# biodatageeks/datafusion-bio-functions

Hardware: AMD Instinct MI355X
Metric: overlap-pairs/sec + probe-rows/sec, IntervalJoinExec 100Mx1M (higher is better)
Workload: dtype int32; 1 GPU; join_100Mx1M_24contigs; probe_rows_per_gpu=100000000, build_rows_per_gpu=1000000, contigs=24, pairs_per_gpu=37210484, parallelism=partition-per-gpu x1, gather=False, build_overlap=True

## Files before the change

datafusion-bio-functions_amd/csrc/ivx_capi.hip:

```cpp
#include "ivx_internal.hpp"
#include "ivx_call.hpp"
#include "ivx_where.hpp"
#include <cstdlib>
#include <atomic>
#include <cstring>
#include <mutex>
#include <new>
#include <thread>
#include <condition_variable>
#include <deque>


void ivx_ctx::join_tail()
{
    if (!tail_pending) return;
    (void)hipStreamWaitEvent(stream, tail_ev, 0);
    tail_pending = false;
}

ivx_status ivx_ctx::get_scratch(int slot, size_t bytes, void **out)
{
    if (tail_pending && slot != WS_SORTHIST && slot != WS_T0 && slot != WS_T1 && slot != WS_T2) join_tail();
    ivx_buf &b = scratch[slot];
    if (sub_plan.valid && ((sub_plan.slots >> slot) & 1)) sub_plan.valid = false;
// ... 409 lines not shown
    w[IVX_STATE_JOIN_FILLS_PLANNED] = ctx->join_fills_planned;
    w[IVX_STATE_SUB_FILLS_PLANNED] = ctx->sub_fills_planned;
    for (int i = 0; i < IVX_NSCRATCH; i++) if (ctx->scratch[i].p) w[IVX_STATE_SCRATCH_HELD] |= 1ull << i;
    {
        std::lock_guard<std::mutex> lk(g_pool_mu);
        for (const PoolBuf &b : g_pool) if (b.device == ctx->device) w[IVX_STATE_POOL_FREE]++;
    }
    for (u32 i = 0; i < n_out && i < (u32)IVX_STATE_WORDS; i++) out[i] = w[i];
    return IVX_OK;
}

extern "C" ivx_status ivx_debug_poison(ivx_ctx *ctx, uint32_t word, int what, uint64_t *slots_written)
{
    if (!ctx) return IVX_ERR_INVALID;
    if (slots_written) *slots_written = 0;
    if (word > 1u) return ctx->fail(IVX_ERR_INVALID, "debug_poison: the word is 0 or 1");
    if (ctx->tail_pending) return ctx->fail(IVX_ERR_INVALID, "debug_poison: a build tail is pending");
    IVX_HIP(ctx, hipSetDevice(ctx->device));
    IVX_HIP(ctx, hipStreamSynchronize(ctx->stream));
    hipStream_t st = ctx->stream;
    const auto fill_host = [word](void *p, size_t bytes) { u32 *q = (u32 *)p; for (size_t i = 0; i < bytes / sizeof(u32); i++) q[i] = word; };
    if (what & IVX_POISON_DROP_PLANS) { ctx->sub_plan.valid = false; ctx->join_plan.valid = false; }
    if (what & IVX_POISON_SCRATCH) {
        const u64 keep = (ctx->sub_plan.valid ? ctx->sub_plan.slots : 0) | (ctx->join_plan.valid ? ctx->join_plan.rows.slots : 0);
        u64 wrote = 0;
        for (int i = 0; i < IVX_NSCRATCH; i++) {
            const ivx_buf &b = ctx->scratch[i];
            if (!b.p || ((keep >> i) & 1)) continue;
            IVX_HIP(ctx, hipMemsetD32Async((hipDeviceptr_t)b.p, (int)word, b.cap / sizeof(u32), st));
            wrote |= 1ull << i;
        }
// ... 1420 lines not shown
```

datafusion-bio-functions_amd/csrc/ivx_device.hpp:

```cpp
#pragma once
#include "ivx_internal.hpp"

__device__ __forceinline__ u32 lane_id() { return __builtin_amdgcn_mbcnt_hi(~0u, __builtin_amdgcn_mbcnt_lo(~0u, 0u)); }

__device__ __forceinline__ u32 mask_rank_from(u64 mask, u32 base)
{
    return __builtin_amdgcn_mbcnt_hi((u32)(mask >> 32), __builtin_amdgcn_mbcnt_lo((u32)mask, base));
}

__device__ __forceinline__ u32 mask_rank(u64 mask)
{
    return __builtin_amdgcn_mbcnt_hi((u32)(mask >> 32), __builtin_amdgcn_mbcnt_lo((u32)mask, 0u));
}

template <typename T>
__device__ __forceinline__ void host_store(T *p, T v) { __hip_atomic_store(p, v, __ATOMIC_RELAXED, __HIP_MEMORY_SCOPE_SYSTEM); }

template <int CTRL, int ROWS>
__device__ __forceinline__ u32 dpp0(u32 v) { return (u32)__builtin_amdgcn_update_dpp(0, (int)v, CTRL, ROWS, 0xf, false); }
__device__ __forceinline__ u32 wave_incl_max32(u32 v)
{
    u32 o;
    o = dpp0<0x111, 0xf>(v); v = o > v ? o : v;
    o = dpp0<0x112, 0xf>(v); v = o > v ? o : v;
// ... 19 lines not shown
#pragma unroll
    for (int d = 1; d < IVX_WAVE; d <<= 1) {
        T o = __shfl_up(v, d, IVX_WAVE);
        if (l >= (u32)d) v += o;
    }
    return v;
}

template <typename T>
__device__ __forceinline__ T wave_sum(T v)
{
#pragma unroll
    for (int d = IVX_WAVE / 2; d > 0; d >>= 1) v += __shfl_xor(v, d, IVX_WAVE);
    return v;
}

template <typename T, int NT>
__device__ __forceinline__ T block_excl_scan(T v, T *lds, T *total)
{
    constexpr int NW = NT / IVX_WAVE;
    const u32 l = lane_id();
    const u32 w = threadIdx.x / IVX_WAVE;
    T inc = wave_incl_scan(v);
    if (l == IVX_WAVE - 1) lds[w] = inc;
    __syncthreads();
    if (threadIdx.x == 0) {
        T run = 0;
#pragma unroll
        for (int i = 0; i < NW; i++) { T t = lds[i]; lds[i] = run; run += t; }
        lds[NW] = run;
// ... 30 lines not shown
```

datafusion-bio-functions_amd/csrc/ivx_grid.hip:

```cpp
#include <cstdlib>
#include "ivx_grid.hpp"
#include "ivx_scan.hpp"

namespace {

constexpr int GT = 256;
constexpr u32 KEYS_IN_LDS = 2048;

__global__ void k_init_keystats(i32 *kmin, i32 *kmax, u32 *kcnt, u32 nkeys, ivx_zero_ranges z)
{
    u32 i = blockIdx.x * blockDim.x + threadIdx.x;
    if (i < nkeys) { kmin[i] = INT32_MAX; kmax[i] = INT32_MIN; kcnt[i] = 0; }
    if (blockIdx.x == 0)
        for (int r = 0; r < 3; r++)
            for (u32 j = threadIdx.x; j < z.n[r]; j += blockDim.x) z.p[r][j] = 0;
    for (u32 j = i; j < z.nbig; j += gridDim.x * blockDim.x) z.big[j] = make_uint4(0u, 0u, 0u, 0u);
}

__global__ __launch_bounds__(GT) void k_keystats(const u32 *__restrict__ key, const i32 *__restrict__ v, u64 n,
                                                 u32 nkeys, i32 *kmin, i32 *kmax, u32 *kcnt, u32 *errflag, u32 vs,
                                                 const i32 *__restrict__ vend, u32 *lenhist)
{
    extern __shared__ i32 sh[];
    __shared__ u32 s_len[33];
    if (lenhist && threadIdx.x < 33) s_len[threadIdx.x] = 0;
    const bool priv = nkeys <= KEYS_IN_LDS;
    if (!priv && lenhist) __syncthreads();
    i32 *smin = sh, *smax = sh + nkeys;
    u32 *scnt = (u32 *)(sh + 2 * nkeys);
    if (priv) {
        for (u32 k = threadIdx.x; k < nkeys; k += GT) { smin[k] = INT32_MAX; smax[k] = INT32_MIN; scnt[k] = 0; }
// ... 17 lines not shown
            clcnt++;
        }
        if (k != ck) { flush(); ck = k; ccnt = 0; cmin = INT32_MAX; cmax = INT32_MIN; }
        cmin = x < cmin ? x : cmin; cmax = x > cmax ? x : cmax; ccnt++;
    }
    flush();
    if (lenhist && clcnt) atomicAdd(&s_len[cl], clcnt);
    if (priv) {
        __syncthreads();
        for (u32 k = threadIdx.x; k < nkeys; k += GT)
            if (scnt[k]) { atomicMin(&kmin[k], smin[k]); atomicMax(&kmax[k], smax[k]); atomicAdd(&kcnt[k], scnt[k]); }
    }
    if (lenhist) {
        __syncthreads();
        if (threadIdx.x < 33 && s_len[threadIdx.x]) atomicAdd(&lenhist[threadIdx.x], s_len[threadIdx.x]);
    }
}

__global__ __launch_bounds__(GT) void k_keystats_sorted(const u32 *__restrict__ key, const i32 *__restrict__ v, u64 n, u32 nkeys,
                                                        i32 *kmin, i32 *kmax, u32 *kcnt, u32 vs)
{
    const u32 k = blockIdx.x * GT + threadIdx.x;
    if (k >= nkeys) return;
    auto lower = [&](u32 x) {
        u64 a = 0, b = n;
        while (a < b) { const u64 m = (a + b) >> 1; if ((key ? key[m] : 0u) < x) a = m + 1; else b = m; }
        return a;
    };
    const u64 lo = lower(k), hi = k + 1 == 0u ? n : lower(k + 1);
    kcnt[k] = (u32)(hi - lo);
// ... 108 lines not shown
}

ivx_status ivx_keystats(ivx_ctx *ctx, const u32 *key, const i32 *v, u64 n, u32 nkeys,
                        i32 *kmin, i32 *kmax, u32 *kcnt, u32 *errflag, u32 vstride)
{
    return ivx_keystats_len(ctx, key, v, n, nkeys, kmin, kmax, kcnt, errflag, vstride, nullptr, nullptr);
}

ivx_status ivx_keystats_len(ivx_ctx *ctx, const u32 *key, const i32 *v, u64 n, u32 nkeys,
                            i32 *kmin, i32 *kmax, u32 *kcnt, u32 *errflag, u32 vstride, const i32 *vend, u32 *lenhist,
                            const ivx_zero_ranges *zero)
{
    hipStream_t st = ctx->stream;
    ivx_zero_ranges z{};
    if (zero) z = *zero;
    u32 igrid = (nkeys + GT - 1) / GT;
    if (z.nbig) { const u32 want = (z.nbig + GT * 8 - 1) / (GT * 8); igrid = igrid > want ? igrid : (want < 256u ? want : 256u); }
    hipLaunchKernelGGL(k_init_keystats, dim3(igrid), dim3(GT), 0, st, kmin, kmax, kcnt, nkeys, z);
    if (n) {
        const u32 grid = ivx_stream_grid(n, GT * 8, 1024);
        const size_t shm = nkeys <= KEYS_IN_LDS ? (size_t)nkeys * 12 : 0;
        hipLaunchKernelGGL(k_keystats, dim3(grid), dim3(GT), shm, st, key, v, n, nkeys, kmin, kmax, kcnt, errflag, vstride, vend, lenhist);
    }
    IVX_HIP(ctx, hipGetLastError());
    return IVX_OK;
}

ivx_status ivx_grid_build(ivx_ctx *ctx, ivx_index *ix, const u32 *key, const i32 *v, u64 n, u32 nkeys, RankGridView *out, bool sorted, u32 vstride)
{
    if (!sorted && vstride != 1) return ctx->fail(IVX_ERR_INVALID, "grid: strided values need a sorted column");
    hipStream_t st = ctx->stream;
    const u64 maxcells = 2 * n + nkeys + 64;
    if (maxcells + 1 >= 0xFFFFFFFFull) return ctx->fail(IVX_ERR_INVALID, "column too large for 32-bit cell ids");
    i32 *origin, *val; u32 *span, *kcnt, *koff, *kbase, *binstart, *hdr;
    IVX_TRY(ivx_index_alloc(ctx, ix, nkeys * sizeof(i32), (void **)&origin));
    IVX_TRY(ivx_index_alloc(ctx, ix, nkeys * sizeof(u32), (void **)&span));
    IVX_TRY(ivx_index_alloc(ctx, ix, nkeys * sizeof(u32), (void **)&kcnt));
    IVX_TRY(ivx_index_alloc(ctx, ix, ((size_t)nkeys + 1) * sizeof(u32), (void **)&koff));
// ... 32 lines not shown
```

datafusion-bio-functions_amd/csrc/ivx_grid.hpp:

```cpp
#pragma once
#include "ivx_device.hpp"

template <int VS = 1>
__device__ __forceinline__ u32 grid_rank_le(const RankGridView &g, u32 sh, u32 k, i32 x)
{
    const u32 cnt = g.kcnt[k];
    const u32 off = g.koff[k];
    if (cnt == 0) return off;
    const i64 d = (i64)x - (i64)g.origin[k];
    if (d < 0) return off;
    if (d > (i64)g.span[k]) return off + cnt;
    const u32 c = g.kbase[k] + (u32)(d >> sh);
    const u32 a = g.binstart[c], b = g.binstart[c + 1];
    u32 r = a;
    for (u32 j = a; j < b; j++) r += g.val[(u64)j * VS] <= x ? 1u : 0u;
    return r;
}

template <int VS = 1>
__device__ __forceinline__ u32 grid_rank_lt(const RankGridView &g, u32 sh, u32 k, i32 x)
{
    if (x == INT32_MIN) return g.koff[k];
    return grid_rank_le<VS>(g, sh, k, x - 1);
}

ivx_status ivx_keystats(ivx_ctx *ctx, const u32 *key, const i32 *v, u64 n, u32 nkeys,
                        i32 *kmin, i32 *kmax, u32 *kcnt, u32 *errflag);
ivx_status ivx_grid_build(ivx_ctx *ctx, ivx_index *ix, const u32 *key, const i32 *v, u64 n, u32 nkeys, RankGridView *out, bool sorted = false,
                          u32 vstride = 1);
ivx_status ivx_keystats(ivx_ctx *ctx, const u32 *key, const i32 *v, u64 n, u32 nkeys,
                        i32 *kmin, i32 *kmax, u32 *kcnt, u32 *errflag, u32 vstride);
struct ivx_zero_ranges { u32 *p[3]; u32 n[3]; uint4 *big = nullptr; u32 nbig = 0; };
ivx_status ivx_keystats_len(ivx_ctx *ctx, const u32 *key, const i32 *v, u64 n, u32 nkeys,
                            i32 *kmin, i32 *kmax, u32 *kcnt, u32 *errflag, u32 vstride, const i32 *vend, u32 *lenhist,
                            const ivx_zero_ranges *zero = nullptr);
```

datafusion-bio-functions_amd/csrc/ivx_internal.hpp:

```cpp
#pragma once
#include <hip/hip_runtime.h>
#include <stdint.h>
#include <atomic>
#include <memory>
#include <string>
#include <vector>
#include "../../include/ivx.h"
#include "../../include/ivx_select.h"
#include "../../include/ivx_nearest.h"

typedef uint8_t u8;
typedef uint32_t u32;
typedef int32_t i32;
typedef uint64_t u64;
typedef int64_t i64;

#define IVX_WAVE 64

struct ivx_buf { void *p = nullptr; size_t cap = 0; };

enum { IVX_NSCRATCH = 56, IVX_NPIN = 4 };

struct ivx_sub_plan {
    bool valid = false;
// ... 124 lines not shown
    WS_GRID0, WS_GRID1, WS_GRID2,
    WS_SORTHIST,
    WS_SA0, WS_SA1, WS_SA2, WS_SB0, WS_SB1, WS_SB2,
    WS_RA0, WS_RA1, WS_RA2, WS_RB0, WS_RB1, WS_RB2,
    WS_T0, WS_T1, WS_T2, WS_T3, WS_T4, WS_T5, WS_T6, WS_T7, WS_T8, WS_T9,
    WS_IN3_KEY, WS_IN3_START, WS_IN3_END, WS_IN3_WEIGHT, WS_IN_KEYLEN,
    WS_IN_TEXTOFF, WS_IN_TEXT
};
static_assert(WS_IN_TEXT < IVX_NSCRATCH, "scratch slot ids must fit the context's slot array");

#ifndef IVX_LSTEP
#define IVX_LSTEP 2
#endif
#define IVX_MAXL (32 / IVX_LSTEP)
#define IVX_SH_MIN 4

struct ivx_ent { i32 s, e; u32 row; };

enum { HDR_SH0 = 0, HDR_NLEV = 1, HDR_NBINS = 2, HDR_CS = 3 , HDR_NREG = 4,
       HDR_RCELLS = 5 , HDR_RMUL_LO = 6, HDR_RMUL_HI = 7 , HDR_LEVCNT = 8 ,
       HDR_FG = 8 + IVX_MAXL , HDR_FBITS = 9 + IVX_MAXL ,
       HDR_PK24 = 10 + IVX_MAXL ,
       HDR_SLOW = 11 + IVX_MAXL ,
       HDR_LBUILD = 12 + IVX_MAXL ,
       HDR_BADKEY = 13 + IVX_MAXL ,
       HDR_WORDS = 14 + IVX_MAXL };
#include "ivx_scalars.hpp"
#define IVX_FBITS_MAX (1u << 24)
#define IVX_MAXREG 255
#define IVX_MAXREG_WIDE 1023
// ... 248 lines not shown
```

datafusion-bio-functions_amd/csrc/ivx_join.hip:

```cpp
#include <cstdlib>
#include <cstring>
#include "ivx_device.hpp"
#include "ivx_grid.hpp"
#include "ivx_join.hpp"

namespace {

constexpr int BT = 256;

constexpr int LB_T = 1024;
constexpr int LB_ROWS = 4;
constexpr u32 LB_TILE = LB_T * LB_ROWS;
constexpr u32 LB_STRIDE = IVX_MAXREG_WIDE + 1;
constexpr u32 LB_CCAP = 8192;
constexpr u32 LB_MAXTILES = 1024;
constexpr int LB_KEEP = (IVX_RP_ECAP + LB_T - 1) / LB_T;
constexpr u64 LB_MIN_ROWS = 1u << 14, LB_MAX_ROWS = (u64)LB_MAXTILES * LB_TILE;
static_assert(LB_STRIDE == LB_T && LB_TILE <= 4096 && LB_CCAP == (1u << IVX_REG_CS_MAX), "k_lbuild_tiles: one table word per thread, 12-bit ranks");
static inline u32 lb_tstride(u32 ntiles) { return ntiles | 1u; }


__device__ __forceinline__ u32 cells_of(u32 cnt, u32 span, u32 sh) { return cnt ? (sh >= 32 ? 1u : (span >> sh) + 1u) : 0u; }

__global__ __launch_bounds__(1024) void k_join_layout(const i32 *kmin, const i32 *kmax, const u32 *kcnt, u32 nkeys, u64 n,
                                                      i32 *origin, u32 *span, u32 *lbase, u32 *hdr, u64 maxcells,
                                                      u32 *kreg, u32 *rkey, const u32 *lenhist, u32 regmax, u32 *fbase, int filter_mode, int lbuild_ok, const u32 *badkey,
                                                      u32 *hmirror)
{
    __shared__ u64 red[1024 / IVX_WAVE + 1];
    __shared__ u32 s_sh0;
    const u32 t = threadIdx.x;
    for (u32 k = t; k < nkeys; k += 1024) {
        u32 c = kcnt[k];
        origin[k] = c ? kmin[k] : 0;
        span[k] = c ? (u32)((i64)kmax[k] - (i64)kmin[k]) : 0u;
    }
    __syncthreads();
    __shared__ u64 s_tot[40];
    __shared__ u64 s_loff[IVX_MAXL + 1];
    const u32 wv = t / IVX_WAVE, ln = lane_id();
    constexpr u32 NWV = 1024 / IVX_WAVE;
    const u64 budget0 = 2 * n + nkeys;
    for (u32 sh = IVX_SH_MIN + wv; sh <= 31; sh += NWV) {
        u64 a = 0;
        for (u32 k = ln; k < nkeys; k += IVX_WAVE) a += cells_of(kcnt[k], span[k], sh);
        a = wave_sum(a);
        if (ln == 0) s_tot[sh] = a;
    }
    __syncthreads();
    __shared__ float s_occ0;
    __shared__ u64 s_cum[34];
    __shared__ float s_cost[32], s_cocc[32];
    __shared__ u32 s_shb;
    if (t <= 32) s_cum[t + 1] = lenhist[t];
    __syncthreads();
    __shared__ u32 s_fg;
    if (t == 0) {
        u32 shb = IVX_SH_MIN;
        while (shb < 31 && s_tot[shb] > budget0) shb++;
        s_shb = shb;
        u32 fg = 0xFFFFFFFFu;
        if (filter_mode != 0 && (u64)nkeys * 34 < IVX_FBITS_MAX / 2) {
            u32 g = IVX_SH_MIN;
            while (g < 31 && s_tot[g] + (u64)nkeys * 34 > IVX_FBITS_MAX) g++;
            const double bits = (double)(s_tot[g] + nkeys);
            double touched = 0.0;
            for (u32 b = 0; b <= 32; b++) touched += (double)s_cum[b + 1] * ((b > g ? (double)(3ull << (b - g)) * 0.25 : 0.0) + 1.5);
            if (n && s_tot[g] + (u64)nkeys * 34 <= IVX_FBITS_MAX && (filter_mode == 2 || touched < 0.15 * bits) && touched < 64.0 * (double)n + 1.0e6) fg = g;
        }
// ... 19 lines not shown
                if (l == 0) { occ0 = occ; cost += 1.f + 2.2f * occ; }
                else if (rows) cost += 8.f + 2.2f * occ * 4.f;
                if (last) break;
                lo_bits = lsh + 1;
            }
        }
        s_cost[t] = cost; s_cocc[t] = occ0;
    }
    __syncthreads();
    if (t == 0) {
        u32 bi = 0;
        for (u32 c = 1; c < 32; c++) if (s_cost[c] < s_cost[bi]) bi = c;
#ifdef IVX_SH_BIAS
        { const int b2 = (int)bi + (IVX_SH_BIAS); bi = b2 < 0 ? 0u : (s_shb + (u32)b2 > 31 ? 31 - s_shb : (u32)b2); }
#endif
        s_sh0 = s_shb + bi; s_occ0 = s_cocc[bi];
    }
    __syncthreads();
    const u32 sh0 = s_sh0;
    u32 nlev = 0;
    for (u32 l = 0; l < IVX_MAXL; l++) { nlev = l + 1; if (sh0 + IVX_LSTEP * l >= 32) break; }
    for (u32 l = wv; l < nlev; l += NWV) {
        const u32 sh = sh0 + IVX_LSTEP * l;
        u64 carry = 0;
        for (u32 k0 = 0; k0 < nkeys; k0 += IVX_WAVE) {
            const u32 k = k0 + ln;
            const u64 c = k < nkeys ? cells_of(kcnt[k], span[k], sh) : 0u;
            const u64 inc = wave_incl_scan(c);
            if (k < nkeys) lbase[(u64)l * nkeys + k] = (u32)(carry + inc - c);
            carry += __shfl(inc, IVX_WAVE - 1, IVX_WAVE);
        }
        if (ln == 0) s_tot[l] = carry;
    }
    __syncthreads();
    if (t == 0) {
        u64 run = 0;
        for (u32 l = 0; l < nlev; l++) { s_loff[l] = run; run += s_tot[l]; }
        hdr[HDR_SH0] = sh0;
        hdr[HDR_NLEV] = nlev;
        hdr[HDR_NBINS] = (u32)(run <= maxcells ? run : maxcells);
    }
    __syncthreads();
    for (u32 l = 1 + wv; l < nlev; l += NWV) {
        const u32 add = (u32)s_loff[l];
        for (u32 k = ln; k < nkeys; k += IVX_WAVE) lbase[(u64)l * nkeys + k] += add;
    }
    for (u32 mid = wv; mid <= 32; mid += NWV) {
        u64 a = 0;
        for (u32 k = ln; k < nkeys; k += IVX_WAVE) {
            const u64 c = cells_of(kcnt[k], span[k], sh0);
            a += mid >= 32 ? (c ? 1u : 0u) : ((c + (1ull << mid) - 1) >> mid);
        }
        a = wave_sum(a);
        if (ln == 0) s_tot[mid] = a;
    }
    __syncthreads();
    u32 clo = 0;
    while (clo < 32 && s_tot[clo] > IVX_MAXREG) clo++;
    if (clo > IVX_REG_CS_MAX && clo <= 32 && s_tot[IVX_REG_CS_MAX] <= IVX_MAXREG2) clo = IVX_REG_CS_MAX;
    u64 R = clo < 32 ? (1ull << clo) : 0;
    bool pow2 = true;
    if (clo < 32 && s_occ0 * (float)R > 0.9f * (float)IVX_RP_ECAP) {
        const float want = 0.85f * (float)IVX_RP_ECAP / s_occ0;
        R = want < 1.f ? 1ull : (u64)want;
        pow2 = false;
    }
    auto regions_for = [&](u64 r) -> u64 {
        u64 a = 0;
        for (u32 k = t; k < nkeys; k += 1024) { const u64 c = cells_of(kcnt[k], span[k], sh0); a += (c + r - 1) / r; }
        return block_sum<u64, 1024>(a, red);
    };
    if (R && nkeys > regmax && regions_for(1ull << 40) > regmax) R = 0;
    if (R) {
        if (!(pow2 && clo < 32 && s_tot[clo] <= regmax)) while (regions_for(R) > regmax) { R *= 2; }
        if (!pow2) {
            u64 mc = 0;
            for (u32 k = t; k < nkeys; k += 1024) { const u64 c = cells_of(kcnt[k], span[k], sh0); mc = c > mc ? c : mc; }
            __shared__ u64 s_mc;
            if (t == 0) s_mc = 0;
            __syncthreads();
            atomicMax((unsigned long long *)&s_mc, (unsigned long long)mc);
            __syncthreads();
            const u64 M = ((1ull << 40) + R - 1) / R;
            if (s_mc * R >= (1ull << 40) || s_mc > (1ull << 63) / M || (R & (R - 1)) == 0) {
                u64 p = 1; while (p * 2 <= R) p *= 2;
                R = p; pow2 = true;
                while (regions_for(R) > regmax) R *= 2;
            }
        }
    }
    u32 cs = 32;
    if (R && pow2) { cs = 0; while ((1ull << cs) < R) cs++; }
    u64 rrun = 0;
    for (u32 k0 = 0; k0 < nkeys; k0 += 1024) {
        const u32 k = k0 + t;
        u64 c = k < nkeys ? cells_of(kcnt[k], span[k], sh0) : 0u;
        c = R ? (c + R - 1) / R : 0;
        u64 tot;
        const u64 ex = block_excl_scan<u64, 1024>(c, red, &tot);
        if (k < nkeys && R) {
            kreg[k] = (u32)(rrun + ex);
            for (u64 r = 0; r < c; r++) rkey[rrun + ex + r] = k;
        }
        rrun += tot;
    }
    {
        const u32 fg = s_fg;
        u64 frun = 0;
        for (u32 k0 = 0; k0 < nkeys; k0 += 1024) {
            const u32 k = k0 + t;
            u64 c = (fg != 0xFFFFFFFFu && k < nkeys && kcnt[k]) ? (u64)(((span[k] >> fg) + 2u + 31u) & ~31u) : 0u;
            u64 tot;
            const u64 ex = block_excl_scan<u64, 1024>(c, red, &tot);
            if (k < nkeys) fbase[k] = (u32)(frun + ex);
            frun += tot;
        }
        if (t == 0) { hdr[HDR_FG] = frun <= IVX_FBITS_MAX ? fg : 0xFFFFFFFFu; hdr[HDR_FBITS] = (u32)frun; }
    }
    if (t == 0) {
        kreg[nkeys] = (u32)rrun;
        hdr[HDR_CS] = pow2 ? cs : 0xFFFFFFFFu;
        hdr[HDR_NREG] = R ? (u32)rrun : 0u;
        hdr[HDR_RCELLS] = (u32)(R > 0xFFFFFFFFull ? 0xFFFFFFFFull : R);
        const u64 M = R ? ((1ull << 40) + R - 1) / R : 0;
        hdr[HDR_RMUL_LO] = (u32)M; hdr[HDR_RMUL_HI] = (u32)(M >> 32);
        hdr[HDR_PK24] = (R && sh0 < 24 && R <= (1ull << (24 - sh0))) ? 1u : 0u;
        hdr[HDR_BADKEY] = *badkey;
        hdr[HDR_LBUILD] = (lbuild_ok && R && R <= LB_CCAP && rrun && rrun <= IVX_MAXREG_WIDE && s_cum[33] == s_cum[sh0 + 1]) ? 1u : 0u;
        static_assert(HDR_WORDS % 2 == 0, "the mirror is written in 8-byte words");
        u32 hv[HDR_WORDS];
#pragma unroll
        for (u32 w = 0; w < HDR_WORDS; w++) hv[w] = hdr[w];
#pragma unroll
        for (u32 w = 0; w < HDR_WORDS; w += 2) host_store((u64 *)hmirror + w / 2, (u64)hv[w] | ((u64)hv[w + 1] << 32));
    }
}

__global__ __launch_bounds__(LB_T) void k_lbuild_tiles(const u32 *__restrict__ key, const i32 *__restrict__ s, const i32 *__restrict__ e, u64 n, u32 nkeys,
                                                     const i32 *origin, const u32 *kreg, u32 *hdr, ivx_ent *__restrict__ rows,
                                                     u32 *__restrict__ tab, u32 tstride, u32 *__restrict__ binstart, u64 nbinwords)
{
    if (hdr[HDR_LBUILD] == 0) {
        for (u64 i = (u64)blockIdx.x * LB_T + threadIdx.x; i < nbinwords; i += (u64)gridDim.x * LB_T) binstart[i] = 0;
        return;
    }
    __shared__ u32 s_cnt[LB_STRIDE];
    __shared__ u32 red[LB_T / IVX_WAVE + 1];
    const u32 t = threadIdx.x;
    s_cnt[t] = 0;
    const u32 sh0 = hdr[HDR_SH0], cs = hdr[HDR_CS];
// ... 384 lines not shown
    IVX_TRY(ivx_index_alloc(ctx, ix, nkeys * sizeof(u32), (void **)&span));
    IVX_TRY(ivx_index_alloc(ctx, ix, nkeys * sizeof(u32), (void **)&kcnt));
    IVX_TRY(ivx_index_alloc(ctx, ix, (size_t)IVX_MAXL * nkeys * sizeof(u32), (void **)&lbase));
    IVX_TRY(ivx_index_alloc(ctx, ix, (maxcells + 1) * sizeof(u32), (void **)&binstart));
    IVX_TRY(ivx_index_alloc(ctx, ix, HDR_WORDS * sizeof(u32), (void **)&hdr));
    IVX_TRY(ivx_index_alloc(ctx, ix, ((size_t)nkeys + 1) * sizeof(u32), (void **)&kreg));
    size_t regcap = (size_t)(n / (IVX_RP_ECAP / 2)) + (size_t)(maxcells >> IVX_REG_CS_MAX) + 2 * (size_t)nkeys + 64;
    regcap = regcap <= IVX_MAXREG + 1 ? (size_t)IVX_MAXREG + 1 : (regcap > (size_t)IVX_MAXREG2 + 1 ? (size_t)IVX_MAXREG2 + 1 : regcap);
    IVX_TRY(ivx_index_alloc(ctx, ix, regcap * sizeof(u32), (void **)&rkey));
    IVX_TRY(ivx_index_alloc(ctx, ix, regcap * sizeof(ivx_regdesc), (void **)&rdesc));
    IVX_TRY(ivx_index_alloc(ctx, ix, (n ? n : 1) * sizeof(ivx_ent), (void **)&ent));
    const size_t fwords = IVX_FBITS_MAX / 32 + 4;
    IVX_TRY(ivx_index_alloc(ctx, ix, nkeys * sizeof(u32), (void **)&fbase));
    IVX_TRY(ivx_index_alloc(ctx, ix, fwords * sizeof(u32), (void **)&fbits));

    i32 *kmin, *kmax; u32 *cellid, *rank, *errflag;
    IVX_TRY(ctx->get_scratch(WS_GRID0, nkeys * sizeof(i32), (void **)&kmin));
    IVX_TRY(ctx->get_scratch(WS_GRID1, nkeys * sizeof(i32), (void **)&kmax));
    const char *benv = getenv("IVX_BUILD");
    const bool lb_try = n >= LB_MIN_ROWS && n <= LB_MAX_ROWS && !(benv && !strcmp(benv, "global"));
    const u32 lb_tiles = lb_try ? (u32)((n + LB_TILE - 1) / LB_TILE) : 0u;
    IVX_TRY(ctx->get_scratch(WS_GRID2, (n ? n : 1) * (lb_try ? sizeof(ivx_ent) : sizeof(u32)), (void **)&cellid));
    const size_t tabbytes = (size_t)lb_tstride(lb_tiles) * LB_STRIDE * sizeof(u32);
    IVX_TRY(ctx->get_scratch(WS_T9, (n ? n : 1) * sizeof(u32) > tabbytes ? (n ? n : 1) * sizeof(u32) : tabbytes, (void **)&rank));
    errflag = ctx->dword<u32>(SC_JOIN_BAD);
    u32 *lenhist = ctx->dword<u32>(SC_JOIN_LENHIST);

    ivx_zero_ranges zr{{errflag, lenhist, hdr}, {1u, (u32)SC_LENHIST_N, (u32)HDR_WORDS}};
    const char *fenv = getenv("IVX_FILTER");
    const int filter_mode = !fenv ? 1 : !strcmp(fenv, "0") ? 0 : !strcmp(fenv, "force") ? 2 : 1;
    static_assert((IVX_FBITS_MAX / 32 + 4) % 4 == 0, "the bitmap is cleared in 16-byte words");
    if (filter_mode) { zr.big = (uint4 *)fbits; zr.nbig = (u32)(fwords / 4); }
    IVX_TRY(ivx_keystats_len(ctx, key, s, n, nkeys, kmin, kmax, kcnt, errflag, 1u, e, lenhist, &zr));
    const u32 grid = ivx_stream_grid(n, BT * 2, 16384);
    u32 *hmirror = ctx->hword<u32>(SC_HDR_MIRROR), *hmirror_d = ctx->hdword<u32>(SC_HDR_MIRROR);
    ctx->hdr_mirror_serial = ix->serial;
    hipLaunchKernelGGL(k_join_layout, dim3(1), dim3(1024), 0, st, kmin, kmax, kcnt, nkeys, n, origin, span, lbase, hdr, maxcells, kreg, rkey, (const u32 *)lenhist, (u32)(regcap - 1), fbase, filter_mode, lb_try ? 1 : 0, (const u32 *)errflag, hmirror_d);
    auto launch_filter = [&]() {
        hipLaunchKernelGGL(k_join_filter, dim3(grid), dim3(BT), 0, st, key, s, e, n, nkeys, (const i32 *)origin, (const u32 *)span, (const u32 *)fbase, (const u32 *)hdr, fbits);
    };
    const bool want_route = ix->kind == IVX_KIND_OVERLAP && n >= (4u << 20);
    overlap = overlap && ctx->overlap && ctx->aux != nullptr && !want_route && n >= (1u << 16);
    if (filter_mode && !overlap) launch_filter();
    hipStream_t tail_st = st;
    struct TailGuard {
        ivx_ctx *c; bool armed = false;
        ~TailGuard() { if (armed) (void)hipStreamSynchronize(c->aux); }
    } guard{ctx};
    bool q_lds = lb_try, q_global = true;
    if (overlap) {
        ctx->join_tail();
        IVX_HIP(ctx, hipEventRecord(ctx->ev_fork, st));
        IVX_HIP(ctx, hipStreamWaitEvent(ctx->aux, ctx->ev_fork, 0));
// ... 77 lines not shown
```

datafusion-bio-functions_amd/csrc/ivx_regions_route.hip:

```cpp
#include "ivx_regions.hpp"

namespace {


constexpr int PA_T = 1024;
#ifndef IVX_PA_I
#define IVX_PA_I 12
#endif
constexpr int PA_I = IVX_PA_I;
constexpr int PA_TILE = PA_T * PA_I;
constexpr u32 NO_REGION = 0xFFFFFFFFu;
constexpr u32 KT_MAX = 256;

struct KeyTab {
    bool lds;
    u32 nkeys, sh0, cs;
    u64 rmul;
};

__device__ __forceinline__ void keytab_load(const JoinIndexView &ix, i32 *s_origin, u32 *s_last, u32 *s_kreg, KeyTab &kt)
{
    kt.nkeys = ix.nkeys; kt.sh0 = ix.hdr[HDR_SH0]; kt.cs = ix.hdr[HDR_CS];
    kt.rmul = (u64)ix.hdr[HDR_RMUL_LO] | ((u64)ix.hdr[HDR_RMUL_HI] << 32);
    kt.lds = ix.nkeys <= KT_MAX;
    if (kt.lds) {
        for (u32 k = threadIdx.x; k < ix.nkeys; k += blockDim.x) {
            s_origin[k] = ix.origin[k];
// ... 1041 lines not shown
```

Before: 38.56 billion overlap-pairs/s.

## Replace atomic build keystats with per-workgroup partials reduced in layout kernel

For small key counts, build-side key statistics (min, max, count, length histogram, bad-key flag) are written as per-workgroup partial arrays instead of being merged with global atomics. The single-block layout kernel then reduces those partials into LDS and reads key tables from LDS. The layout kernel also folds the level offsets into the prefix scan and writes the header in one pass, and the filter bitmap clear moves to a separate kernel that skips work when the filter is disabled. This is meant to remove global atomic contention and the init pass on the build path, at the cost of more template and launch complexity.

```diff
diff --git a/datafusion-bio-functions_amd/csrc/ivx_capi.hip b/datafusion-bio-functions_amd/csrc/ivx_capi.hip
--- a/datafusion-bio-functions_amd/csrc/ivx_capi.hip
+++ b/datafusion-bio-functions_amd/csrc/ivx_capi.hip
@@ -447,7 +447,7 @@
 {
     if (!ctx) return IVX_ERR_INVALID;
     if (slots_written) *slots_written = 0;
-    if (word > 1u) return ctx->fail(IVX_ERR_INVALID, "debug_poison: the word is 0 or 1");
+    if (word > 1u && word != 0xFFFFFFFFu) return ctx->fail(IVX_ERR_INVALID, "debug_poison: the word is 0 or 1 (or all ones)");
     if (ctx->tail_pending) return ctx->fail(IVX_ERR_INVALID, "debug_poison: a build tail is pending");
     IVX_HIP(ctx, hipSetDevice(ctx->device));
     IVX_HIP(ctx, hipStreamSynchronize(ctx->stream));
diff --git a/datafusion-bio-functions_amd/csrc/ivx_device.hpp b/datafusion-bio-functions_amd/csrc/ivx_device.hpp
--- a/datafusion-bio-functions_amd/csrc/ivx_device.hpp
+++ b/datafusion-bio-functions_amd/csrc/ivx_device.hpp
@@ -57,6 +57,20 @@
     for (int d = IVX_WAVE / 2; d > 0; d >>= 1) v += __shfl_xor(v, d, IVX_WAVE);
     return v;
 }
+template <typename T>
+__device__ __forceinline__ T wave_min(T v)
+{
+#pragma unroll
+    for (int d = IVX_WAVE / 2; d > 0; d >>= 1) { const T o = __shfl_xor(v, d, IVX_WAVE); v = o < v ? o : v; }
+    return v;
+}
+template <typename T>
+__device__ __forceinline__ T wave_max(T v)
+{
+#pragma unroll
+    for (int d = IVX_WAVE / 2; d > 0; d >>= 1) { const T o = __shfl_xor(v, d, IVX_WAVE); v = o > v ? o : v; }
+    return v;
+}
 
 template <typename T, int NT>
 __device__ __forceinline__ T block_excl_scan(T v, T *lds, T *total)
diff --git a/datafusion-bio-functions_amd/csrc/ivx_grid.hip b/datafusion-bio-functions_amd/csrc/ivx_grid.hip
--- a/datafusion-bio-functions_amd/csrc/ivx_grid.hip
+++ b/datafusion-bio-functions_amd/csrc/ivx_grid.hip
@@ -14,7 +14,6 @@
     if (blockIdx.x == 0)
         for (int r = 0; r < 3; r++)
             for (u32 j = threadIdx.x; j < z.n[r]; j += blockDim.x) z.p[r][j] = 0;
-    for (u32 j = i; j < z.nbig; j += gridDim.x * blockDim.x) z.big[j] = make_uint4(0u, 0u, 0u, 0u);
 }
 
 __global__ __launch_bounds__(GT) void k_keystats(const u32 *__restrict__ key, const i32 *__restrict__ v, u64 n,
@@ -62,6 +61,55 @@
     if (lenhist) {
         __syncthreads();
         if (threadIdx.x < 33 && s_len[threadIdx.x]) atomicAdd(&lenhist[threadIdx.x], s_len[threadIdx.x]);
+    }
+}
+
+__global__ __launch_bounds__(GT) void k_keystats_part(const u32 *__restrict__ key, const i32 *__restrict__ v, const i32 *__restrict__ vend,
+                                                      u64 n, u32 nkeys, u32 *__restrict__ part)
+{
+    __shared__ i32 smin[KT_MAX], smax[KT_MAX];
+    __shared__ u32 scnt[KT_MAX], s_len[33], s_bad;
+    for (u32 k = threadIdx.x; k < nkeys; k += GT) { smin[k] = INT32_MAX; smax[k] = INT32_MIN; scnt[k] = 0; }
+    if (threadIdx.x < 33) s_len[threadIdx.x] = 0;
+    if (threadIdx.x == 0) s_bad = 0;
+    __syncthreads();
+    u32 ck = 0xFFFFFFFFu, ccnt = 0; i32 cmin = INT32_MAX, cmax = INT32_MIN;
+    u32 cl = 0xFFFFFFFFu, clcnt = 0;
+    auto flush = [&]() {
+        if (!ccnt) return;
+        atomicMin(&smin[ck], cmin); atomicMax(&smax[ck], cmax); atomicAdd(&scnt[ck], ccnt);
+    };
+    auto row = [&](u32 k, i32 x, i32 xe) {
+        if (k >= nkeys) { s_bad = 1u; return; }
+        const i64 len = (i64)xe - (i64)x;
+        const u32 c = len <= 0 ? 0u : 64u - (u32)__clzll((u64)len);
+        if (c != cl) { if (clcnt) atomicAdd(&s_len[cl], clcnt); cl = c; clcnt = 0; }
+        clcnt++;
+        if (k != ck) { flush(); ck = k; ccnt = 0; cmin = INT32_MAX; cmax = INT32_MIN; }
+        cmin = x < cmin ? x : cmin; cmax = x > cmax ? x : cmax; ccnt++;
+    };
+    const u64 stride = (u64)gridDim.x * GT;
+    u64 i = (u64)blockIdx.x * GT + threadIdx.x;
+    for (; i + 3 * stride < n; i += 4 * stride) {
+        u32 k4[4]; i32 x4[4], e4[4];
+#pragma unroll
+        for (int q = 0; q < 4; q++) { const u64 j = i + (u64)q * stride; k4[q] = key ? key[j] : 0u; x4[q] = v[j]; e4[q] = vend[j]; }
+#pragma unroll
+        for (int q = 0; q < 4; q++) row(k4[q], x4[q], e4[q]);
+    }
+    for (; i < n; i += stride) row(key ? key[i] : 0u, v[i], vend[i]);
+    flush();
+    if (clcnt) atomicAdd(&s_len[cl], clcnt);
+    __syncthreads();
+    const u32 items = ivx_ks_items(nkeys);
+    for (u32 it = threadIdx.x; it < items; it += GT) {
+        u32 w;
+        if (it < nkeys) w = (u32)smin[it];
+        else if (it < 2 * nkeys) w = (u32)smax[it - nkeys];
+        else if (it < 3 * nkeys) w = scnt[it - 2 * nkeys];
+        else if (it < 3 * nkeys + 33) w = s_len[it - 3 * nkeys];
+        else w = s_bad;
+        part[(u64)it * gridDim.x + blockIdx.x] = w;
     }
 }
 
@@ -200,14 +248,23 @@
     hipStream_t st = ctx->stream;
     ivx_zero_ranges z{};
     if (zero) z = *zero;
-    u32 igrid = (nkeys + GT - 1) / GT;
-    if (z.nbig) { const u32 want = (z.nbig + GT * 8 - 1) / (GT * 8); igrid = igrid > want ? igrid : (want < 256u ? want : 256u); }
+    const u32 igrid = (nkeys + GT - 1) / GT;
     hipLaunchKernelGGL(k_init_keystats, dim3(igrid), dim3(GT), 0, st, kmin, kmax, kcnt, nkeys, z);
     if (n) {
         const u32 grid = ivx_stream_grid(n, GT * 8, 1024);
         const size_t shm = nkeys <= KEYS_IN_LDS ? (size_t)nkeys * 12 : 0;
         hipLaunchKernelGGL(k_keystats, dim3(grid), dim3(GT), shm, st, key, v, n, nkeys, kmin, kmax, kcnt, errflag, vstride, vend, lenhist);
     }
+    IVX_HIP(ctx, hipGetLastError());
+    return IVX_OK;
+}
+
+u32 ivx_keystats_part_grid(u64 n) { return n ? ivx_stream_grid(n, GT * IVX_KP_ROWS, IVX_KP_MAXWG) : 0u; }
+
+ivx_status ivx_keystats_part(ivx_ctx *ctx, const u32 *key, const i32 *v, const i32 *vend, u64 n, u32 nkeys, u32 *part, u32 nwg)
+{
+    if (nkeys > KT_MAX || nwg != ivx_keystats_part_grid(n)) return ctx->fail(IVX_ERR_INVALID, "keystats_part: key count or grid");
+    if (nwg) hipLaunchKernelGGL(k_keystats_part, dim3(nwg), dim3(GT), 0, ctx->stream, key, v, vend, n, nkeys, part);
     IVX_HIP(ctx, hipGetLastError());
     return IVX_OK;
 }
diff --git a/datafusion-bio-functions_amd/csrc/ivx_grid.hpp b/datafusion-bio-functions_amd/csrc/ivx_grid.hpp
--- a/datafusion-bio-functions_amd/csrc/ivx_grid.hpp
+++ b/datafusion-bio-functions_amd/csrc/ivx_grid.hpp
@@ -30,7 +30,16 @@
                           u32 vstride = 1);
 ivx_status ivx_keystats(ivx_ctx *ctx, const u32 *key, const i32 *v, u64 n, u32 nkeys,
                         i32 *kmin, i32 *kmax, u32 *kcnt, u32 *errflag, u32 vstride);
-struct ivx_zero_ranges { u32 *p[3]; u32 n[3]; uint4 *big = nullptr; u32 nbig = 0; };
+struct ivx_zero_ranges { u32 *p[3]; u32 n[3]; };
 ivx_status ivx_keystats_len(ivx_ctx *ctx, const u32 *key, const i32 *v, u64 n, u32 nkeys,
                             i32 *kmin, i32 *kmax, u32 *kcnt, u32 *errflag, u32 vstride, const i32 *vend, u32 *lenhist,
                             const ivx_zero_ranges *zero = nullptr);
+constexpr u32 ivx_ks_items(u32 nkeys) { return 3u * nkeys + 34u; }
+#ifndef IVX_KP_ROWS
+#define IVX_KP_ROWS 16
+#endif
+#ifndef IVX_KP_MAXWG
+#define IVX_KP_MAXWG 256
+#endif
+u32 ivx_keystats_part_grid(u64 n);
+ivx_status ivx_keystats_part(ivx_ctx *ctx, const u32 *key, const i32 *v, const i32 *vend, u64 n, u32 nkeys, u32 *part, u32 nwg);
diff --git a/datafusion-bio-functions_amd/csrc/ivx_internal.hpp b/datafusion-bio-functions_amd/csrc/ivx_internal.hpp
--- a/datafusion-bio-functions_amd/csrc/ivx_internal.hpp
+++ b/datafusion-bio-functions_amd/csrc/ivx_internal.hpp
@@ -162,6 +162,7 @@
 #endif
 #define IVX_MAXL (32 / IVX_LSTEP)
 #define IVX_SH_MIN 4
+constexpr u32 KT_MAX = 256;
 
 struct ivx_ent { i32 s, e; u32 row; };
 
diff --git a/datafusion-bio-functions_amd/csrc/ivx_join.hip b/datafusion-bio-functions_amd/csrc/ivx_join.hip
--- a/datafusion-bio-functions_amd/csrc/ivx_join.hip
+++ b/datafusion-bio-functions_amd/csrc/ivx_join.hip
@@ -22,37 +22,103 @@
 
 __device__ __forceinline__ u32 cells_of(u32 cnt, u32 span, u32 sh) { return cnt ? (sh >= 32 ? 1u : (span >> sh) + 1u) : 0u; }
 
-__global__ __launch_bounds__(1024) void k_join_layout(const i32 *kmin, const i32 *kmax, const u32 *kcnt, u32 nkeys, u64 n,
+template <bool KLDS>
+__global__ __launch_bounds__(1024) void k_join_layout(const i32 *kmin, const i32 *kmax, u32 *kcnt, u32 nkeys, u64 n,
                                                       i32 *origin, u32 *span, u32 *lbase, u32 *hdr, u64 maxcells,
                                                       u32 *kreg, u32 *rkey, const u32 *lenhist, u32 regmax, u32 *fbase, int filter_mode, int lbuild_ok, const u32 *badkey,
-                                                      u32 *hmirror)
+                                                      u32 *hmirror, const u32 *__restrict__ part, u32 npart)
 {
     __shared__ u64 red[1024 / IVX_WAVE + 1];
-    __shared__ u32 s_sh0;
+    __shared__ u32 s_sh0, s_nlev, s_nbins, s_bad;
+    __shared__ i32 s_org[KLDS ? KT_MAX : 1];
+    __shared__ u32 s_spn[KLDS ? KT_MAX : 1], s_kc[KLDS ? KT_MAX : 1];
+    __shared__ u64 s_cum[34];
     const u32 t = threadIdx.x;
-    for (u32 k = t; k < nkeys; k += 1024) {
-        u32 c = kcnt[k];
-        origin[k] = c ? kmin[k] : 0;
-        span[k] = c ? (u32)((i64)kmax[k] - (i64)kmin[k]) : 0u;
+    const u32 wv = t / IVX_WAVE, ln = lane_id();
+    constexpr u32 NWV = 1024 / IVX_WAVE;
+    auto cnt_of = [&](u32 k) -> u32 { if constexpr (KLDS) return s_kc[k]; else return kcnt[k]; };
+    auto span_of = [&](u32 k) -> u32 { if constexpr (KLDS) return s_spn[k]; else return span[k]; };
+    if constexpr (KLDS) {
+        if (part) {
+            constexpr u32 KP_LW = IVX_KP_MAXWG / IVX_WAVE, KP_B = 8;
+            static_assert(IVX_KP_MAXWG % IVX_WAVE == 0, "whole wavefronts of partial words");
+            const u32 items = ivx_ks_items(nkeys);
+            for (u32 it0 = wv; it0 < items; it0 += NWV * KP_B) {
+                u32 w[KP_B][KP_LW];
+#pragma unroll
+                for (u32 b = 0; b < KP_B; b++) {
+                    const u32 it = it0 + b * NWV;
+                    const u32 ident = it < nkeys ? (u32)INT32_MAX : it < 2 * nkeys ? (u32)INT32_MIN : 0u;
+#pragma unroll
+                    for (u32 q = 0; q < KP_LW; q++) {
+                        const u32 j = ln + q * IVX_WAVE;
+                        w[b][q] = (it < items && j < npart) ? part[(u64)it * npart + j] : ident;
+                    }
+                }
+#pragma unroll
+                for (u32 b = 0; b < KP_B; b++) {
+                    const u32 it = it0 + b * NWV;
+                    if (it >= items) break;
+                    if (it < nkeys) {
+                        i32 m = (i32)w[b][0];
+#pragma unroll
+                        for (u32 q = 1; q < KP_LW; q++) m = (i32)w[b][q] < m ? (i32)w[b][q] : m;
+                        m = wave_min(m);
+                        if (ln == 0) s_org[it] = m;
+                    } else if (it < 2 * nkeys) {
+                        i32 m = (i32)w[b][0];
+#pragma unroll
+                        for (u32 q = 1; q < KP_LW; q++) m = (i32)w[b][q] > m ? (i32)w[b][q] : m;
+                        m = wave_max(m);
+                        if (ln == 0) s_spn[it - nkeys] = (u32)m;
+                    } else {
+                        u32 a = 0;
+#pragma unroll
+                        for (u32 q = 0; q < KP_LW; q++) a += w[b][q];
+                        a = wave_sum(a);
+                        if (ln == 0) {
+                            if (it < 3 * nkeys) s_kc[it - 2 * nkeys] = a;
+                            else if (it < 3 * nkeys + 33) s_cum[it - 3 * nkeys + 1] = a;
+                            else s_bad = a ? 1u : 0u;
+                        }
+                    }
+                }
+            }
+            __syncthreads();
+        }
+        if (t < nkeys) {
+            const u32 c = part ? s_kc[t] : kcnt[t];
+            const i32 lo = part ? s_org[t] : kmin[t], hi = part ? (i32)s_spn[t] : kmax[t];
+            const i32 o = c ? lo : 0;
+            const u32 w = c ? (u32)((i64)hi - (i64)lo) : 0u;
+            s_kc[t] = c; s_org[t] = o; s_spn[t] = w;
+            origin[t] = o; span[t] = w;
+            if (part) kcnt[t] = c;
+        }
+    } else {
+        for (u32 k = t; k < nkeys; k += 1024) {
+            u32 c = kcnt[k];
+            origin[k] = c ? kmin[k] : 0;
+            span[k] = c ? (u32)((i64)kmax[k] - (i64)kmin[k]) : 0u;
+        }
+    }
+    if (!(KLDS && part)) {
+        if (t <= 32) s_cum[t + 1] = lenhist[t];
+        if (t == 0) s_bad = *badkey;
     }
     __syncthreads();
     __shared__ u64 s_tot[40];
     __shared__ u64 s_loff[IVX_MAXL + 1];
-    const u32 wv = t / IVX_WAVE, ln = lane_id();
-    constexpr u32 NWV = 1024 / IVX_WAVE;
     const u64 budget0 = 2 * n + nkeys;
-    for (u32 sh = IVX_SH_MIN + wv; sh <= 31; sh += NWV) {
+    for (u32 sh = IVX_SH_MIN + wv; sh <= 32; sh += NWV) {
         u64 a = 0;
-        for (u32 k = ln; k < nkeys; k += IVX_WAVE) a += cells_of(kcnt[k], span[k], sh);
+        for (u32 k = ln; k < nkeys; k += IVX_WAVE) a += cells_of(cnt_of(k), span_of(k), sh);
         a = wave_sum(a);
         if (ln == 0) s_tot[sh] = a;
     }
-    __syncthreads();
     __shared__ float s_occ0;
-    __shared__ u64 s_cum[34];
     __shared__ float s_cost[32], s_cocc[32];
     __shared__ u32 s_shb;
-    if (t <= 32) s_cum[t + 1] = lenhist[t];
     __syncthreads();
     __shared__ u32 s_fg;
     if (t == 0) {
@@ -102,41 +168,32 @@
 #ifdef IVX_SH_BIAS
         { const int b2 = (int)bi + (IVX_SH_BIAS); bi = b2 < 0 ? 0u : (s_shb + (u32)b2 > 31 ? 31 - s_shb : (u32)b2); }
 #endif
-        s_sh0 = s_shb + bi; s_occ0 = s_cocc[bi];
-    }
-    __syncthreads();
-    const u32 sh0 = s_sh0;
-    u32 nlev = 0;
-    for (u32 l = 0; l < IVX_MAXL; l++) { nlev = l + 1; if (sh0 + IVX_LSTEP * l >= 32) break; }
+        const u32 sh0 = s_shb + bi;
+        s_sh0 = sh0; s_occ0 = s_cocc[bi];
+        u32 nlev = 0;
+        for (u32 l = 0; l < IVX_MAXL; l++) { nlev = l + 1; if (sh0 + IVX_LSTEP * l >= 32) break; }
+        u64 run = 0;
+        for (u32 l = 0; l < nlev; l++) { const u32 lsh = sh0 + IVX_LSTEP * l; s_loff[l] = run; run += s_tot[lsh < 32 ? lsh : 32]; }
+        s_nlev = nlev;
+        s_nbins = (u32)(run <= maxcells ? run : maxcells);
+    }
+    __syncthreads();
+    const u32 sh0 = s_sh0, nlev = s_nlev;
     for (u32 l = wv; l < nlev; l += NWV) {
         const u32 sh = sh0 + IVX_LSTEP * l;
-        u64 carry = 0;
+        u64 carry = s_loff[l];
         for (u32 k0 = 0; k0 < nkeys; k0 += IVX_WAVE) {
             const u32 k = k0 + ln;
-            const u64 c = k < nkeys ? cells_of(kcnt[k], span[k], sh) : 0u;
+            const u64 c = k < nkeys ? cells_of(cnt_of(k), span_of(k), sh) : 0u;
             const u64 inc = wave_incl_scan(c);
             if (k < nkeys) lbase[(u64)l * nkeys + k] = (u32)(carry + inc - c);
             carry += __shfl(inc, IVX_WAVE - 1, IVX_WAVE);
         }
-        if (ln == 0) s_tot[l] = carry;
-    }
-    __syncthreads();
-    if (t == 0) {
-        u64 run = 0;
-        for (u32 l = 0; l < nlev; l++) { s_loff[l] = run; run += s_tot[l]; }
-        hdr[HDR_SH0] = sh0;
-        hdr[HDR_NLEV] = nlev;
-        hdr[HDR_NBINS] = (u32)(run <= maxcells ? run : maxcells);
-    }
-    __syncthreads();
-    for (u32 l = 1 + wv; l < nlev; l += NWV) {
-        const u32 add = (u32)s_loff[l];
-        for (u32 k = ln; k < nkeys; k += IVX_WAVE) lbase[(u64)l * nkeys + k] += add;
     }
     for (u32 mid = wv; mid <= 32; mid += NWV) {
         u64 a = 0;
         for (u32 k = ln; k < nkeys; k += IVX_WAVE) {
-            const u64 c = cells_of(kcnt[k], span[k], sh0);
+            const u64 c = cells_of(cnt_of(k), span_of(k), sh0);
             a += mid >= 32 ? (c ? 1u : 0u) : ((c + (1ull << mid) - 1) >> mid);
         }
         a = wave_sum(a);
@@ -155,7 +212,7 @@
     }
     auto regions_for = [&](u64 r) -> u64 {
         u64 a = 0;
-        for (u32 k = t; k < nkeys; k += 1024) { const u64 c = cells_of(kcnt[k], span[k], sh0); a += (c + r - 1) / r; }
+        for (u32 k = t; k < nkeys; k += 1024) { const u64 c = cells_of(cnt_of(k), span_of(k), sh0); a += (c + r - 1) / r; }
         return block_sum<u64, 1024>(a, red);
     };
     if (R && nkeys > regmax && regions_for(1ull << 40) > regmax) R = 0;
@@ -163,7 +220,7 @@
         if (!(pow2 && clo < 32 && s_tot[clo] <= regmax)) while (regions_for(R) > regmax) { R *= 2; }
         if (!pow2) {
             u64 mc = 0;
-            for (u32 k = t; k < nkeys; k += 1024) { const u64 c = cells_of(kcnt[k], span[k], sh0); mc = c > mc ? c : mc; }
+            for (u32 k = t; k < nkeys; k += 1024) { const u64 c = cells_of(cnt_of(k), span_of(k), sh0); mc = c > mc ? c : mc; }
             __shared__ u64 s_mc;
             if (t == 0) s_mc = 0;
             __syncthreads();
@@ -182,7 +239,7 @@
     u64 rrun = 0;
     for (u32 k0 = 0; k0 < nkeys; k0 += 1024) {
         const u32 k = k0 + t;
-        u64 c = k < nkeys ? cells_of(kcnt[k], span[k], sh0) : 0u;
+        u64 c = k < nkeys ? cells_of(cnt_of(k), span_of(k), sh0) : 0u;
         c = R ? (c + R - 1) / R : 0;
         u64 tot;
         const u64 ex = block_excl_scan<u64, 1024>(c, red, &tot);
@@ -192,36 +249,43 @@
         }
         rrun += tot;
     }
-    {
-        const u32 fg = s_fg;
-        u64 frun = 0;
-        for (u32 k0 = 0; k0 < nkeys; k0 += 1024) {
-            const u32 k = k0 + t;
-            u64 c = (fg != 0xFFFFFFFFu && k < nkeys && kcnt[k]) ? (u64)(((span[k] >> fg) + 2u + 31u) & ~31u) : 0u;
-            u64 tot;
-            const u64 ex = block_excl_scan<u64, 1024>(c, red, &tot);
-            if (k < nkeys) fbase[k] = (u32)(frun + ex);
-            frun += tot;
-        }
-        if (t == 0) { hdr[HDR_FG] = frun <= IVX_FBITS_MAX ? fg : 0xFFFFFFFFu; hdr[HDR_FBITS] = (u32)frun; }
+    const u32 fg = s_fg;
+    u64 frun = 0;
+    for (u32 k0 = 0; k0 < nkeys; k0 += 1024) {
+        const u32 k = k0 + t;
+        u64 c = (fg != 0xFFFFFFFFu && k < nkeys && cnt_of(k)) ? (u64)(((span_of(k) >> fg) + 2u + 31u) & ~31u) : 0u;
+        u64 tot;
+        const u64 ex = block_excl_scan<u64, 1024>(c, red, &tot);
+        if (k < nkeys) fbase[k] = (u32)(frun + ex);
+        frun += tot;
     }
     if (t == 0) {
         kreg[nkeys] = (u32)rrun;
-        hdr[HDR_CS] = pow2 ? cs : 0xFFFFFFFFu;
-        hdr[HDR_NREG] = R ? (u32)rrun : 0u;
-        hdr[HDR_RCELLS] = (u32)(R > 0xFFFFFFFFull ? 0xFFFFFFFFull : R);
-        const u64 M = R ? ((1ull << 40) + R - 1) / R : 0;
-        hdr[HDR_RMUL_LO] = (u32)M; hdr[HDR_RMUL_HI] = (u32)(M >> 32);
-        hdr[HDR_PK24] = (R && sh0 < 24 && R <= (1ull << (24 - sh0))) ? 1u : 0u;
-        hdr[HDR_BADKEY] = *badkey;
-        hdr[HDR_LBUILD] = (lbuild_ok && R && R <= LB_CCAP && rrun && rrun <= IVX_MAXREG_WIDE && s_cum[33] == s_cum[sh0 + 1]) ? 1u : 0u;
         static_assert(HDR_WORDS % 2 == 0, "the mirror is written in 8-byte words");
         u32 hv[HDR_WORDS];
 #pragma unroll
-        for (u32 w = 0; w < HDR_WORDS; w++) hv[w] = hdr[w];
+        for (u32 w = 0; w < HDR_WORDS; w++) hv[w] = 0u;
+        hv[HDR_SH0] = sh0; hv[HDR_NLEV] = nlev; hv[HDR_NBINS] = s_nbins;
+        hv[HDR_FG] = frun <= IVX_FBITS_MAX ? fg : 0xFFFFFFFFu; hv[HDR_FBITS] = (u32)frun;
+        hv[HDR_CS] = pow2 ? cs : 0xFFFFFFFFu;
+        hv[HDR_NREG] = R ? (u32)rrun : 0u;
+        hv[HDR_RCELLS] = (u32)(R > 0xFFFFFFFFull ? 0xFFFFFFFFull : R);
+        const u64 M = R ? ((1ull << 40) + R - 1) / R : 0;
+        hv[HDR_RMUL_LO] = (u32)M; hv[HDR_RMUL_HI] = (u32)(M >> 32);
+        hv[HDR_PK24] = (R && sh0 < 24 && R <= (1ull << (24 - sh0))) ? 1u : 0u;
+        hv[HDR_BADKEY] = s_bad;
+        hv[HDR_LBUILD] = (lbuild_ok && R && R <= LB_CCAP && rrun && rrun <= IVX_MAXREG_WIDE && s_cum[33] == s_cum[sh0 + 1]) ? 1u : 0u;
+#pragma unroll
+        for (u32 w = 0; w < HDR_WORDS; w++) hdr[w] = hv[w];
 #pragma unroll
         for (u32 w = 0; w < HDR_WORDS; w += 2) host_store((u64 *)hmirror + w / 2, (u64)hv[w] | ((u64)hv[w + 1] << 32));
     }
+}
+
+__global__ __launch_bounds__(BT) void k_join_filter_clear(const u32 *hdr, uint4 *fbits, u32 nquads)
+{
+    if (hdr[HDR_FG] == 0xFFFFFFFFu) return;
+    for (u32 j = blockIdx.x * BT + threadIdx.x; j < nquads; j += gridDim.x * BT) fbits[j] = make_uint4(0u, 0u, 0u, 0u);
 }
 
 __global__ __launch_bounds__(LB_T) void k_lbuild_tiles(const u32 *__restrict__ key, const i32 *__restrict__ s, const i32 *__restrict__ e, u64 n, u32 nkeys,
@@ -636,9 +700,16 @@
     IVX_TRY(ivx_index_alloc(ctx, ix, nkeys * sizeof(u32), (void **)&fbase));
     IVX_TRY(ivx_index_alloc(ctx, ix, fwords * sizeof(u32), (void **)&fbits));
 
-    i32 *kmin, *kmax; u32 *cellid, *rank, *errflag;
-    IVX_TRY(ctx->get_scratch(WS_GRID0, nkeys * sizeof(i32), (void **)&kmin));
-    IVX_TRY(ctx->get_scratch(WS_GRID1, nkeys * sizeof(i32), (void **)&kmax));
+    const char *kenv = getenv("IVX_KEYSTATS");
+    const bool ks_part = nkeys <= KT_MAX && !(kenv && !strcmp(kenv, "atomic"));
+    const u32 ks_wg = ks_part ? ivx_keystats_part_grid(n) : 0u;
+    i32 *kmin = nullptr, *kmax = nullptr; u32 *cellid, *rank, *errflag, *kpart = nullptr;
+    if (ks_part) {
+        IVX_TRY(ctx->get_scratch(WS_GRID0, (size_t)ivx_ks_items(nkeys) * (ks_wg ? ks_wg : 1u) * sizeof(u32), (void **)&kpart));
+    } else {
+        IVX_TRY(ctx->get_scratch(WS_GRID0, nkeys * sizeof(i32), (void **)&kmin));
+        IVX_TRY(ctx->get_scratch(WS_GRID1, nkeys * sizeof(i32), (void **)&kmax));
+    }
     const char *benv = getenv("IVX_BUILD");
     const bool lb_try = n >= LB_MIN_ROWS && n <= LB_MAX_ROWS && !(benv && !strcmp(benv, "global"));
     const u32 lb_tiles = lb_try ? (u32)((n + LB_TILE - 1) / LB_TILE) : 0u;
@@ -648,17 +719,25 @@
     errflag = ctx->dword<u32>(SC_JOIN_BAD);
     u32 *lenhist = ctx->dword<u32>(SC_JOIN_LENHIST);
 
-    ivx_zero_ranges zr{{errflag, lenhist, hdr}, {1u, (u32)SC_LENHIST_N, (u32)HDR_WORDS}};
     const char *fenv = getenv("IVX_FILTER");
     const int filter_mode = !fenv ? 1 : !strcmp(fenv, "0") ? 0 : !strcmp(fenv, "force") ? 2 : 1;
-    static_assert((IVX_FBITS_MAX / 32 + 4) % 4 == 0, "the bitmap is cleared in 16-byte words");
-    if (filter_mode) { zr.big = (uint4 *)fbits; zr.nbig = (u32)(fwords / 4); }
-    IVX_TRY(ivx_keystats_len(ctx, key, s, n, nkeys, kmin, kmax, kcnt, errflag, 1u, e, lenhist, &zr));
+    if (ks_part) {
+        IVX_TRY(ivx_keystats_part(ctx, key, s, e, n, nkeys, kpart, ks_wg));
+    } else {
+        const ivx_zero_ranges zr{{errflag, lenhist, nullptr}, {1u, (u32)SC_LENHIST_N, 0u}};
+        IVX_TRY(ivx_keystats_len(ctx, key, s, n, nkeys, kmin, kmax, kcnt, errflag, 1u, e, lenhist, &zr));
+    }
     const u32 grid = ivx_stream_grid(n, BT * 2, 16384);
     u32 *hmirror = ctx->hword<u32>(SC_HDR_MIRROR), *hmirror_d = ctx->hdword<u32>(SC_HDR_MIRROR);
     ctx->hdr_mirror_serial = ix->serial;
-    hipLaunchKernelGGL(k_join_layout, dim3(1), dim3(1024), 0, st, kmin, kmax, kcnt, nkeys, n, origin, span, lbase, hdr, maxcells, kreg, rkey, (const u32 *)lenhist, (u32)(regcap - 1), fbase, filter_mode, lb_try ? 1 : 0, (const u32 *)errflag, hmirror_d);
+#define IVX_LAYOUT_LAUNCH(KLDS_) hipLaunchKernelGGL(k_join_layout<KLDS_>, dim3(1), dim3(1024), 0, st, (const i32 *)kmin, (const i32 *)kmax, kcnt, nkeys, n, origin, span, lbase, hdr, maxcells, kreg, rkey, \
+        (const u32 *)lenhist, (u32)(regcap - 1), fbase, filter_mode, lb_try ? 1 : 0, (const u32 *)errflag, hmirror_d, (const u32 *)kpart, ks_wg)
+    if (nkeys <= KT_MAX) IVX_LAYOUT_LAUNCH(true); else IVX_LAYOUT_LAUNCH(false);
+#undef IVX_LAYOUT_LAUNCH
+    static_assert((IVX_FBITS_MAX / 32 + 4) % 4 == 0, "the bitmap is cleared in 16-byte words");
     auto launch_filter = [&]() {
+        const u32 nquads = (u32)(fwords / 4);
+        hipLaunchKernelGGL(k_join_filter_clear, dim3(ivx_stream_grid(nquads, BT * 8, 256)), dim3(BT), 0, st, (const u32 *)hdr, (uint4 *)fbits, nquads);
         hipLaunchKernelGGL(k_join_filter, dim3(grid), dim3(BT), 0, st, key, s, e, n, nkeys, (const i32 *)origin, (const u32 *)span, (const u32 *)fbase, (const u32 *)hdr, fbits);
     };
     const bool want_route = ix->kind == IVX_KIND_OVERLAP && n >= (4u << 20);
diff --git a/datafusion-bio-functions_amd/csrc/ivx_regions_route.hip b/datafusion-bio-functions_amd/csrc/ivx_regions_route.hip
--- a/datafusion-bio-functions_amd/csrc/ivx_regions_route.hip
+++ b/datafusion-bio-functions_amd/csrc/ivx_regions_route.hip
@@ -10,7 +10,6 @@
 constexpr int PA_I = IVX_PA_I;
 constexpr int PA_TILE = PA_T * PA_I;
 constexpr u32 NO_REGION = 0xFFFFFFFFu;
-constexpr u32 KT_MAX = 256;
 
 struct KeyTab {
     bool lds;
```

Result: no change. 38.46 billion overlap-pairs/s (-0.3%).
